# xj361685640/fdtd3d

Hardware: AMD Instinct MI355X
Metric: Mcells/sec (whole node), 3D vacuum 1024^3 grid at 1/2/4/8 MI355X (higher is better)
Workload: dtype fp32; 1 GPU; model=fdtd3d 3D Yee leapfrog, vacuum, point dipole (BASELINE.json headline), grid=1024x1024x1024, global_batch=1, seq_len=1073741824, parallelism=domain-decomposition 1x1x1 (dp1-equivalent ranks), backend=hip

## Files before the change

### fdtd3d_amd/csrc/capi.h

```cpp
#pragma once

#include <stdint.h>

extern "C" {
int fdtd_abi_version();

int fdtd_update_e3d_f32(float* ex, float* ey, float* ez, const float* hx, const float* hy, const float* hz,
                        const float* cbx, const float* cby, const float* cbz, double cb, int nx, int ny, int nz,
                        const int* boxes, int xchunk, void* stream);
int fdtd_update_h3d_f32(float* hx, float* hy, float* hz, const float* ex, const float* ey, const float* ez,
                        const float* dbx, const float* dby, const float* dbz, double db, int nx, int ny, int nz,
                        const int* boxes, int xchunk, void* stream);
int fdtd_update_e3d_f64(double* ex, double* ey, double* ez, const double* hx, const double* hy, const double* hz,
                        const double* cbx, const double* cby, const double* cbz, double cb, int nx, int ny, int nz,
                        const int* boxes, int xchunk, void* stream);
int fdtd_update_h3d_f64(double* hx, double* hy, double* hz, const double* ex, const double* ey, const double* ez,
                        const double* dbx, const double* dby, const double* dbz, double db, int nx, int ny, int nz,
                        const int* boxes, int xchunk, void* stream);
int fdtd_update_e3d_v4_f32(float* ex, float* ey, float* ez, const float* hx, const float* hy, const float* hz,
                           const float* cbx, const float* cby, const float* cbz, double cb, int nx, int ny, int nz,
                           const int* boxes, int xchunk, void* stream);
int fdtd_update_e3d_cpml_v4_f32(float* ex, float* ey, float* ez, const float* hx, const float* hy, const float* hz,
                                const float* cbx, const float* cby, const float* cbz, double cb, int nx, int ny,
                                int nz, const int* boxes, int xchunk, const void* const* cp, const int* ci,
// ... 21 lines not shown
int fdtd_inc_e_f32(float* einc, const float* hinc, int n, double c, double src, void* stream);
int fdtd_inc_e_f64(double* einc, const double* hinc, int n, double c, double src, void* stream);
int fdtd_inc_h_f32(const float* einc, float* hinc, int n, double c, void* stream);
int fdtd_inc_h_f64(const double* einc, double* hinc, int n, double c, void* stream);
int fdtd_tfsf_apply_f32(float* target, const long long* off, const long long* i0, const float* w0, const float* w1,
                        const float* coef, const int* ijk, int n, const float* inc, const int* box, void* stream);
int fdtd_tfsf_apply_f64(double* target, const long long* off, const long long* i0, const double* w0,
                        const double* w1, const double* coef, const int* ijk, int n, const double* inc,
                        const int* box, void* stream);
int fdtd_update_h3d_v4_f32(float* hx, float* hy, float* hz, const float* ex, const float* ey, const float* ez,
                           const float* dbx, const float* dby, const float* dbz, double db, int nx, int ny, int nz,
                           const int* boxes, int xchunk, void* stream);
int fdtd_fused3d_f32(const float* const* ein, const float* const* hin, float* const* eout, float* const* hout,
                     const float* const* cbs, const float* const* dbs, double cb, double db, int nx, int ny, int nz,
                     const int* boxes, int xchunk, long long src_off, int src_comp, double src_val, void* s);
int fdtd_fused3d_f64(const double* const* ein, const double* const* hin, double* const* eout,
                     double* const* hout, const double* const* cbs, const double* const* dbs, double cb, double db,
                     int nx, int ny, int nz, const int* boxes, int xchunk, long long src_off, int src_comp,
                     double src_val, void* s);
int fdtd_fused3d_v4_f32(const float* const* ein, const float* const* hin, float* const* eout, float* const* hout,
                        const float* const* cbs, const float* const* dbs, double cb, double db, int nx, int ny,
                        int nz, const int* boxes, int xchunk, long long src_off, int src_comp, double src_val,
                        void* s);

struct FdtdTbOpts {
  int vec;
  int rows;
  int xcd;
  int mrows;
  int variant;
  int mr_shape;
  int dr_shape;
  int half64;
};
int fdtd_tb_opts_size();
int fdtd_tb3d_v4_f32(const float* const* ein, const float* const* hin, float* const* eout, float* const* hout,
                     const float* const* cbs, const float* const* dbs, double cb, double db, int nx, int ny, int nz,
                     const int* boxes, const int* obox, int xchunk, int steps, const int* src, const double* src_vals,
                     const FdtdTbOpts* opts, void* stream);
int fdtd_tb_max_steps();
int fdtd_tb3d_ext_f32(const float* const* ein, const float* const* hin, float* const* eout, float* const* hout,
                      const void* ce4, const int* ebox, const void* ch4, const int* hbox, double cb, double db,
                      int nx, int ny, int nz, const int* boxes, const int* obox, int xchunk, int steps,
                      const int* src, const double* src_vals, const void* tf, const float* gtab,
                      const FdtdTbOpts* opts, void* stream);
int fdtd_box_pack_f32(float* const* fields, float* buf, int ncomp, int ny, int nz, const int* box, void* s);
int fdtd_box_pack_f64(double* const* fields, double* buf, int ncomp, int ny, int nz, const int* box, void* s);
int fdtd_box_unpack_f32(float* const* fields, const float* buf, int ncomp, int ny, int nz, const int* box, void* s);
int fdtd_box_unpack_f64(double* const* fields, const double* buf, int ncomp, int ny, int nz, const int* box, void* s);
int fdtd_box_xfer_f32(float* const* src, float* const* dst, int ncomp, int ny, int nz, const int* box, void* s);
int fdtd_box_xfer_f64(double* const* src, double* const* dst, int ncomp, int ny, int nz, const int* box, void* s);
int fdtd_tb3d_amp_f32(const float* const* ein, const float* const* hin, float* const* eout, float* const* hout,
                      double cb, double db, int nx, int ny, int nz, const int* boxes, const int* obox, int xchunk,
                      int steps, const int* src, const double* src_vals, float* const* amp, const int* aboxes,
                      double accuracy, unsigned* counts, const FdtdTbOpts* opts, void* stream);
int fdtd_tb3d_drude_f32(const float* const* ein, const float* const* hin, float* const* eout, float* const* hout,
                        double cb, double db, int nx, int ny, int nz, const int* boxes, const int* obox, int xchunk,
                        int steps, const int* src, const double* src_vals, const int* bbox, void* const* sin,
                        void* const* sout, const void* lut, int nid, double cbd, const FdtdTbOpts* opts, void* stream);
int fdtd_tfdev_size();
int fdtd_tfsf_pass_f32(float* einc, float* hinc, int n, double ce, double ch, const double* src_vals, int steps,
                       int reach, int nE, int nH, const int* I0, const float* W0, const float* W1, const float* C,
                       float* gtab, void* stream);
int fdtd_tfsf_table_f32(const float* esrc, const float* hsrc, float* einc, float* hinc, int n, double ce, double ch,
                        const double* src_vals, int steps, int reach, int nE, int nH, const int* I0, const float* W0,
                        const float* W1, const float* C, float* gtab, void* stream);
// ... 108 lines not shown
```

### fdtd3d_amd/csrc/host_native.cpp

```cpp
#include "host_native.h"

#include <algorithm>
#include <cmath>
#include <cstdio>
#include <cstring>
#include <fstream>
#include <limits>
#include <tuple>

namespace fdtd {

double halo_cost(const Int3& size, const Int3& topo) {
  double chunk[3];
  for (int a = 0; a < 3; ++a) chunk[a] = (double)size[a] / topo[a];
  double cost = 0;
  for (int a = 0; a < 3; ++a) {
    if (topo[a] <= 1) continue;
    double other = 1;
    for (int b = 0; b < 3; ++b)
      if (b != a) other *= chunk[b];
    cost += (topo[a] > 2 ? 2 : 1) * other;
  }
  return cost;
}

Int3 optimal_topology(const Int3& size, int p, const std::vector<int>& axes) {
  auto allowed = [&](int a) { return std::find(axes.begin(), axes.end(), a) != axes.end(); };
  Int3 best = {p, 1, 1};
  bool have = false;
  std::tuple<double, int, int, int, int> bestkey;
  for (int pass = 0; pass < 2 && !have; ++pass)
  for (int px = 1; px <= p; ++px) {
    if (p % px) continue;
// ... 234 lines not shown
                                                                         const int* act, int T, int* out, int cap) {
  fdtd::Box6 a, k, dm;
  for (int q = 0; q < 6; ++q) {
    a[q] = alloc[q];
    k[q] = K[q];
    dm[q] = Dm[q];
  }
  const bool ac[3] = {act[0] != 0, act[1] != 0, act[2] != 0};
  std::vector<std::vector<fdtd::Box6>> shells;
  std::vector<fdtd::Box6> copy;
  if (T < 1 || !fdtd::hybrid_windows(a, k, dm, T, ac, {size[0], size[1], size[2]}, shells, copy)) return -1;
  int n = 0;
  auto put = [&](const std::vector<fdtd::Box6>& v) {
    if (n + 1 + 6 * (int)v.size() > cap) return false;
    out[n++] = (int)v.size();
    for (const auto& b : v)
      for (int q = 0; q < 6; ++q) out[n++] = b[q];
    return true;
  };
  for (const auto& v : shells)
    if (!put(v)) return -2;
  if (!put(copy)) return -2;
  return n;
}

extern "C" __attribute__((visibility("default"))) void fdtd_optimal_topology(const int* size, int nprocs,
                                                                                const int* axes, int naxes,
                                                                                int* out) {
  fdtd::Int3 s = {size[0], size[1], size[2]};
  std::vector<int> ax(axes, axes + naxes);
  fdtd::Int3 t = fdtd::optimal_topology(s, nprocs, ax);
  for (int a = 0; a < 3; ++a) out[a] = t[a];
}
```

### fdtd3d_amd/csrc/tb3d_mr.h

```cpp
#pragma once

#include <cstdio>
#include <cstdlib>
#include <type_traits>

#include "capi.h"
#include "common.h"
#include "tfsf_dev.h"

namespace tb3d {

constexpr int TBW = 16;

template <int V>
struct VT;
template <>
struct VT<1> {
  typedef float f __attribute__((ext_vector_type(1)));
  typedef unsigned u __attribute__((ext_vector_type(1)));
};
template <>
struct VT<2> {
  typedef float f __attribute__((ext_vector_type(2)));
  typedef unsigned u __attribute__((ext_vector_type(2)));
};
template <>
struct VT<4> {
  typedef float f __attribute__((ext_vector_type(4)));
  typedef unsigned u __attribute__((ext_vector_type(4)));
};

__device__ __forceinline__ float lane_up(float v) {
  return __builtin_bit_cast(float, __builtin_amdgcn_update_dpp(0, __builtin_bit_cast(int, v), 0x138, 0xf, 0xf, false));
}
__device__ __forceinline__ float lane_dn(float v) {
  return __builtin_bit_cast(float, __builtin_amdgcn_update_dpp(0, __builtin_bit_cast(int, v), 0x130, 0xf, 0xf, false));
}

struct TbSrc {
  float v[8];
// ... 83 lines not shown
}

template <int V>
__device__ __forceinline__ typename VT<V>::f zm1(const typename VT<V>::f& v, float s) {
  typename VT<V>::f r;
  r[0] = s;
#pragma unroll
  for (int q = 1; q < V; ++q) r[q] = v[q - 1];
  return r;
}
template <int V>
__device__ __forceinline__ typename VT<V>::f zp1(const typename VT<V>::f& v, float s) {
  typename VT<V>::f r;
#pragma unroll
  for (int q = 0; q < V - 1; ++q) r[q] = v[q + 1];
  r[V - 1] = s;
  return r;
}

template <int V>
struct F3 {
  typename VT<V>::f x, y, z;
};

template <int T, int V, int R, int FX, int PFD, bool DEFER, int NW>
__global__ __launch_bounds__(64 * NW) void k_tb3d_mr(
    const float* __restrict__ exi, const float* __restrict__ eyi, const float* __restrict__ ezi,
    const float* __restrict__ hxi, const float* __restrict__ hyi, const float* __restrict__ hzi,
    float* __restrict__ exo, float* __restrict__ eyo, float* __restrict__ ezo,
    float* __restrict__ hxo, float* __restrict__ hyo, float* __restrict__ hzo,
    const float4* __restrict__ ce4, const float4* __restrict__ ch4, Box3 BE, Box3 BH, float cb,
    float db, int nx, int ny, int nz, Box3 bex, Box3 bey, Box3 bez, Box3 bhx, Box3 bhy, Box3 bhz, Box3 O,
    int xchunk, int src_i, int src_j, int src_k, int src_comp, TbSrc sv, int xcd_swz,
    const TfDev* __restrict__ tf, const float* __restrict__ gtab, AmpDev amp, DrDev dr) {
  constexpr int PC = FX & 3;
  constexpr bool TFS = FX & 4;
  constexpr bool AMP = FX & 8;
  constexpr bool DRU = FX & 16;
  static_assert(!AMP || (FX == 8 && V == 1 && T <= 3), "amplitude mode: scalar lanes, alone, T <= 3");
  static_assert(!DRU || FX == 16, "Drude box: alone");
  static_assert(V == 1 || !FX, "sparse coefficients / TF/SF: scalar lanes");
  constexpr bool PCE = PC & 1, PCH = PC & 2;
  static_assert(R * V <= 4, "mask bit field holds 7 boxes x R rows x V cells");
  typedef typename VT<V>::f vec;
  constexpr int HL = (T + V - 1) / V;
  constexpr int TBZ = (64 - 2 * HL) * V;
  constexpr int ROWS = NW * R;
  constexpr unsigned VM = (1u << V) - 1u;
  __shared__ vec sX[2][4][NW][64];
  const int lane = threadIdx.x;
  const int w = __builtin_amdgcn_readfirstlane(threadIdx.y);
  typedef const __attribute__((address_space(4))) TfDev* TfPtr;
  const TfPtr TFc = (TfPtr)tf;

  int tz = blockIdx.x, ty = blockIdx.y, tx = blockIdx.z;
  if (xcd_swz & 1) {
    const int gx = gridDim.x, gy = gridDim.y;
    const int n = gx * gy * (int)gridDim.z;
    const int p = blockIdx.x + gx * (blockIdx.y + gy * blockIdx.z);
    const int n8 = n & ~7;
    const int q = p < n8 ? (p & 7) * (n8 >> 3) + (p >> 3) : p;
    const int pz = (xcd_swz >> 8) & 0xff, py = (xcd_swz >> 16) & 0xff;
    if (pz > 0 && py > 0) {
      tx = q / (gx * gy);
      const int r = q - tx * gx * gy;
      const int band = r / (py * gx);
      const int h = min(py, gy - band * py);
      const int rb = r - band * py * gx;
      const int col = rb / (pz * h);
      const int wdt = min(pz, gx - col * pz);
      const int e = rb - col * pz * h;
      tz = col * pz + e % wdt;
      ty = band * py + e / wdt;
    } else {
      tz = q % gx;
      ty = (q / gx) % gy;
      tx = q / (gx * gy);
    }
  }
  const int kb = (O.lo[2] & ~(V - 1)) - HL * V + TBZ * tz + V * lane;
  const int jw = O.lo[1] - T + (ROWS - 2 * T) * ty + R * w;
  const int i0 = O.lo[0] + tx * xchunk;
  const int i1 = min(i0 + xchunk, O.hi[0]);
  const bool kin = kb >= 0 && kb < nz;
  const bool lane_own = lane >= HL && lane < 64 - HL;
  const size_t plane = (size_t)ny * nz;
  unsigned roff[R];
  unsigned mbits = 0;
  const Box3* bx[7] = {&bex, &bey, &bez, &bhx, &bhy, &bhz, &O};
#pragma unroll
  for (int r = 0; r < R; ++r) {
    const int j = jw + r;
    const int t = R * w + r;
    const bool ld_ok = kin && j >= 0 && j < ny;
    roff[r] = ld_ok ? (unsigned)(j * nz + kb) * 4u : 0xF0000000u;
    const bool own = ld_ok && lane_own && t >= T && t < ROWS - T;
#pragma unroll
    for (int n = 0; n < 7; ++n) {
      const bool ok = n < 6 ? ld_ok : own;
      mbits |= (ok ? kmaskv<V>(*bx[n], j, kb) : 0u) << ((r * 7 + n) * V);
    }
  }
  const int rdn = w > 0 ? w - 1 : 0;
  const int rup = w < NW - 1 ? w + 1 : NW - 1;
  const vec zero = (vec)(0.f);
  const vec cbv = (vec)(cb), dbv = (vec)(db);
  unsigned upd_bits = 0;
#pragma unroll
  for (int r = 0; r < R; ++r) upd_bits |= ((1u << (6 * V)) - 1u) << (r * 7 * V);
  const bool tile_all = __all((mbits & upd_bits) == upd_bits);

  unsigned eoff[R], hoff[R];
  unsigned inb = 0;
  const int bez_n = BE.hi[2] - BE.lo[2], bhz_n = BH.hi[2] - BH.lo[2];
  const size_t eplane = (size_t)(BE.hi[1] - BE.lo[1]) * bez_n * 16u;
  const size_t hplane = (size_t)(BH.hi[1] - BH.lo[1]) * bhz_n * 16u;
// ... 551 lines not shown
      for (int r = 0; r < R; ++r) Hs[r] = Hc[r];
    } else {
      if constexpr (TFS)
        store_plane(X, Ep[T - 1], Hc);
      else
        store_plane(X, En, Hc);
    }
  }
  if (DEFER) {
    F3<V> Es[R];
#pragma unroll
    for (int r = 0; r < R; ++r) Es[r] = Ep[T - 1][r];
    store_plane(i1 + T - 1, Es, Hs);
  }
  };
  if (tile_all && !(xcd_swz & 2))
    run(std::true_type{});
  else
    run(std::false_type{});
  if constexpr (AMP) {
#pragma unroll
    for (int l = 0; l < T; ++l) {
      unsigned v = acnt[l];
#pragma unroll
      for (int d = 32; d > 0; d >>= 1) v += __shfl_xor(v, d, 64);
      if (lane == 0 && v) atomicAdd(amp.counts + l, v);
    }
  }
}


inline FdtdTbOpts tb_opts(const FdtdTbOpts* p) {
  FdtdTbOpts o = { 0,  0,  0,  0,  4,  0,  0,
                   1};
  if (!p) return o;
  o.vec = (p->vec == 2 || p->vec == 4) ? p->vec : 0;
  o.rows = (p->rows == 1 || p->rows == 2) ? p->rows : 0;
  o.xcd = p->xcd ? 1 : 0;
  o.mrows = (p->mrows == 1 || p->mrows == 2) ? p->mrows : 0;
  o.variant = p->variant & 15;
  o.mr_shape = (p->mr_shape == 1 || p->mr_shape == 2) ? p->mr_shape : 0;
  o.dr_shape = p->dr_shape == 1 ? 1 : 0;
  o.half64 = p->half64 ? 1 : 0;
  return o;
}

inline int tb_patch_bits() {
  static const int bits = [] {
    const char* e = getenv("FDTD3D_TB_PATCH");
    int pz = 0, py = 0;
    if (e && sscanf(e, "%dx%d", &pz, &py) == 2 && pz > 0 && py > 0 && pz < 256 && py < 256)
      return (pz << 8) | (py << 16);
    return 0;
  }();
  return bits;
}

template <int T, int V, int R, int FX, int NW = TBW>
int launch_tb_mr(const FdtdTbOpts& o, const float* const* ein, const float* const* hin, float* const* eout,
                 float* const* hout, const float4* ce4, const float4* ch4, const Box3& BE, const Box3& BH, float cb,
                 float db, int nx, int ny, int nz, const Box3* b, const Box3& O, int xchunk, const int* src,
                 const TbSrc& sv, const TfDev* tf, const float* gtab, const AmpDev& amp, hipStream_t s,
                 const DrDev& dr = DrDev{}) {
  constexpr int HL = (T + V - 1) / V;
  constexpr int TBZ = (64 - 2 * HL) * V;
  dim3 grid(cdiv(O.hi[2] - (O.lo[2] & ~(V - 1)), TBZ), cdiv(O.hi[1] - O.lo[1], NW * R - 2 * T),
            cdiv(O.hi[0] - O.lo[0], xchunk));
  const int noallin = (o.variant >> 3) & 1;
  const int swz = (o.variant & 4) ? (1 | (noallin << 1) | tb_patch_bits()) : (noallin << 1);
#define MR_LAUNCH(PFD, DEFER)                                                                                 \
  k_tb3d_mr<T, V, R, FX, PFD, DEFER, NW><<<grid, dim3(64, NW), 0, s>>>(                                     \
      ein[0], ein[1], ein[2], hin[0], hin[1], hin[2], eout[0], eout[1], eout[2], hout[0], hout[1], hout[2], \
      ce4, ch4, BE, BH, cb, db, nx, ny, nz, b[0], b[1], b[2], b[3], b[4], b[5],                             \
      O, xchunk, src[0], src[1], src[2], src[3], sv, swz, tf, gtab, amp, dr)
  if constexpr (FX != 0) {
    MR_LAUNCH(1, false);
  } else {
    switch (o.variant & 3) {
      case 0: MR_LAUNCH(1, false); break;
      case 1: MR_LAUNCH(1, true); break;
      case 2: MR_LAUNCH(2, false); break;
      default: MR_LAUNCH(2, true); break;
    }
  }
#undef MR_LAUNCH
  FDTD_RETURN_LAUNCH_STATUS();
}

}
```

### fdtd3d_amd/csrc/yee3d_tb.hip

```cpp

#include <cstdio>
#include <cstdlib>
#include <type_traits>

#include "common.h"

#include "tb3d_mr.h"

namespace {

using namespace tb3d;

template <int T, int V, int R, bool PERCELL>
__global__ __launch_bounds__(64 * TBW) void k_tb3d(
    const float* __restrict__ exi, const float* __restrict__ eyi, const float* __restrict__ ezi,
    const float* __restrict__ hxi, const float* __restrict__ hyi, const float* __restrict__ hzi,
    float* __restrict__ exo, float* __restrict__ eyo, float* __restrict__ ezo,
    float* __restrict__ hxo, float* __restrict__ hyo, float* __restrict__ hzo,
    const float* __restrict__ cbx, const float* __restrict__ cby, const float* __restrict__ cbz,
    const float* __restrict__ dbx, const float* __restrict__ dby, const float* __restrict__ dbz, float cb,
    float db, int nx, int ny, int nz, Box3 bex, Box3 bey, Box3 bez, Box3 bhx, Box3 bhy, Box3 bhz, Box3 O,
    int xchunk, int src_i, int src_j, int src_k, int src_comp, TbSrc sv, int xcd_swz) {
  typedef typename VT<V>::f vec;
  constexpr bool PF = V == 2;
// ... 103 lines not shown
      }
      const int ph = pe - 1;
      const float ey_k3 = lane_dn(Ep[l].y[0]);
      const float ex_k3 = lane_dn(Ep[l].x[0]);
      F3<V> Hn;
      const vec chx = coef(dbx, bhx, ph, mhx, mchx, dbv);
      Hn.x = Hp[l].x + chx * ((zp1<V>(Ep[l].y, ey_k3) - Ep[l].y) - (ez_jn - Ep[l].z));
      const vec chy = coef(dby, bhy, ph, mhy, mchy, dbv);
      Hn.y = Hp[l].y + chy * ((En.z - Ep[l].z) - (zp1<V>(Ep[l].x, ex_k3) - Ep[l].x));
      const vec chz = coef(dbz, bhz, ph, mhz, mchz, dbv);
      Hn.z = Hp[l].z + chz * ((ex_jn - Ep[l].x) - (En.y - Ep[l].y));
      Ec = Ep[l];
      Ep[l] = En;
      Hp[l] = Hc;
      Hc = Hn;
    }
    if (mo) {
      const int pe = X - T + 1;
      if (pe >= i0 && pe < i1) {
        bst<V>(plane_rsrc(exo, pe, nx, plane), row, En.x, mo);
        bst<V>(plane_rsrc(eyo, pe, nx, plane), row, En.y, mo);
        bst<V>(plane_rsrc(ezo, pe, nx, plane), row, En.z, mo);
      }
      const int ph = X - T;
      if (ph >= i0 && ph < i1) {
        bst<V>(plane_rsrc(hxo, ph, nx, plane), row, Hc.x, mo);
        bst<V>(plane_rsrc(hyo, ph, nx, plane), row, Hc.y, mo);
        bst<V>(plane_rsrc(hzo, ph, nx, plane), row, Hc.z, mo);
      }
    }
  }
}

int g_num_cus = 0;
int pick_xchunk(long long tiles_yz, int nxo, int T, int wg_per_cu = 1) {
  if (g_num_cus <= 0) {
    int dev = 0, n = 0;
    if (hipGetDevice(&dev) == hipSuccess &&
        hipDeviceGetAttribute(&n, hipDeviceAttributeMultiprocessorCount, dev) == hipSuccess && n > 0)
      g_num_cus = n;
    else
      g_num_cus = 256;
  }
  if (nxo <= 0) return 1;
  const long long slots = (long long)g_num_cus * wg_per_cu;
  auto search = [&](int cap, long long* rounds_out) {
    long long best_cost = -1, best_rounds = 1;
    int best = nxo;
    for (int k = 1; k <= 256; ++k) {
      const int xc = (nxo + k - 1) / k;
      if (xc > cap) continue;
      const long long chunks = (nxo + xc - 1) / xc;
      const long long rounds = (tiles_yz * chunks + slots - 1) / slots;
      const long long cost = rounds * (xc + 2LL * T);
      if (best_cost < 0 || cost < best_cost) {
        best_cost = cost;
        best = xc;
        best_rounds = rounds;
      }
      if (xc == 1) break;
    }
    *rounds_out = best_rounds;
    return best;
  };
  long long rounds = 1;
  const int best = search(nxo, &rounds);
  static int cap = -1;
  if (cap < 0) {
    const char* e = getenv("FDTD3D_TB_XCAP");
    cap = (e && atoi(e) > 0) ? atoi(e) : 192;
  }
  if (rounds >= 2 && best > cap) return search(cap, &rounds);
  return best;
}

template <int T, int V, int R, bool PERCELL>
int launch_tb(const float* const* ein, const float* const* hin, float* const* eout, float* const* hout,
              const float* const* cbs, const float* const* dbs, float cb, float db, int nx, int ny, int nz,
              const Box3* b, const Box3& O, int xchunk, const int* src, const TbSrc& sv, hipStream_t s, int xcd) {
  constexpr int HL = (T + V - 1) / V;
  constexpr int TBZ = (64 / R - 2 * HL) * V;
  dim3 grid(cdiv(O.hi[2] - (O.lo[2] & ~(V - 1)), TBZ), cdiv(O.hi[1] - O.lo[1], TBW * R - 2 * T),
            cdiv(O.hi[0] - O.lo[0], xchunk));
  k_tb3d<T, V, R, PERCELL><<<grid, dim3(64, TBW), 0, s>>>(
      ein[0], ein[1], ein[2], hin[0], hin[1], hin[2], eout[0], eout[1], eout[2], hout[0], hout[1], hout[2],
      cbs[0], cbs[1], cbs[2], dbs[0], dbs[1], dbs[2], cb, db, nx, ny, nz, b[0], b[1], b[2], b[3], b[4], b[5], O,
      xchunk, src[0], src[1], src[2], src[3], sv, xcd);
  FDTD_RETURN_LAUNCH_STATUS();
}

template <int T, int V, int R>
int launch_tb_pc(bool pc, const float* const* ein, const float* const* hin, float* const* eout,
                 float* const* hout, const float* const* cbs, const float* const* dbs, float cb, float db, int nx,
                 int ny, int nz, const Box3* b, const Box3& O, int xchunk, const int* src, const TbSrc& sv,
                 hipStream_t s, int xcd) {
  return pc ? launch_tb<T, V, R, true>(ein, hin, eout, hout, cbs, dbs, cb, db, nx, ny, nz, b, O, xchunk, src, sv, s,
                                       xcd)
            : launch_tb<T, V, R, false>(ein, hin, eout, hout, cbs, dbs, cb, db, nx, ny, nz, b, O, xchunk, src, sv,
                                        s, xcd);
}

constexpr int MR_AUTO_ROWS = 2;

const int kNoBox[6] = {0, 0, 0, 0, 0, 0};
static int tb_amp_shape() {
  static const int v = [] {
// ... 16 lines not shown
      if (o.dr_shape == 1) return launch_tb_mr<T, 1, 1, 16, 16>(MR_ARGS);
      return launch_tb_mr<T, 1, 2, 16, 8>(MR_ARGS);
    }
    return (int)hipErrorInvalidValue;
  }
  if (fx == 8) {
    if constexpr (T <= 3) {
      if (o.mr_shape == 1) return launch_tb_mr<T, 1, 4, 8, 8>(MR_ARGS);
      if (tb_amp_shape() == 2) return launch_tb_mr<T, 1, 2, 8, 8>(MR_ARGS);
      return launch_tb_mr<T, 1, 2, 8>(MR_ARGS);
    }
    return (int)hipErrorInvalidValue;
  }
  if constexpr (T <= 5) {
    switch (fx) {
      case 1: return launch_tb_mr<T, 1, 2, 1>(MR_ARGS);
      case 2: return launch_tb_mr<T, 1, 2, 2>(MR_ARGS);
      case 3: return launch_tb_mr<T, 1, 2, 3>(MR_ARGS);
      case 4: return launch_tb_mr<T, 1, 2, 4>(MR_ARGS);
      case 5: return launch_tb_mr<T, 1, 2, 5>(MR_ARGS);
      case 6: return launch_tb_mr<T, 1, 2, 6>(MR_ARGS);
      case 7: return launch_tb_mr<T, 1, 2, 7>(MR_ARGS);
    }
  } else {
    if (fx) return (int)hipErrorInvalidValue;
  }
  if (o.mr_shape == 1) return launch_tb_mr<T, 1, 4, 0, 8>(MR_ARGS);
  if constexpr (T <= 5)
    if (o.mr_shape == 2) return launch_tb_mr<T, 1, 2, 0, 8>(MR_ARGS);
  return launch_tb_mr<T, 1, 2, 0>(MR_ARGS);
#undef MR_ARGS
}

int tb_mr_xchunk(int fx, const FdtdTbOpts& o, const Box3& O, int steps) {
  const long long gz = cdiv(O.hi[2] - O.lo[2], 64 - 2 * steps);
  const bool amp16 = fx == 8 && o.mr_shape != 1 && tb_amp_shape() == 2;
  const bool rows16 = fx == 16 || amp16 || (fx == 0 && o.mr_shape == 2 && steps <= 5);
  const long long gy = cdiv(O.hi[1] - O.lo[1], (rows16 ? 16 : TBW * 2) - 2 * steps);
  return pick_xchunk(gz * gy, O.hi[0] - O.lo[0], steps, ((fx == 0 && o.mr_shape >= 1) || amp16) ? 2 : 1);
}

int tb_mr_dispatch(int fx, const FdtdTbOpts& o, const float* const* ein, const float* const* hin,
                   float* const* eout, float* const* hout, const float4* ce4, const float4* ch4, const Box3& BE,
                   const Box3& BH, float cb, float db, int nx, int ny, int nz, const Box3* b, const Box3& O,
                   int xchunk, int steps, const int* src, const TbSrc& sv, const TfDev* tf, const float* gtab,
                   const AmpDev& amp, hipStream_t s, const DrDev& dr = DrDev{}) {
  if (xchunk <= 0 && (fx & 4)) {
    static const int tfx = [] {
      const char* e = getenv("FDTD3D_TF_XCHUNK");
      return e ? atoi(e) : 0;
    }();
    if (tfx > 0) xchunk = tfx;
  }
  if (xchunk <= 0) xchunk = tb_mr_xchunk(fx, o, O, steps);
#define MR_ARGS \
  fx, o, ein, hin, eout, hout, ce4, ch4, BE, BH, cb, db, nx, ny, nz, b, O, xchunk, src, sv, tf, gtab, amp, s, dr
  switch (steps) {
    case 1: return launch_tb_mr_sel<1>(MR_ARGS);
    case 2: return launch_tb_mr_sel<2>(MR_ARGS);
    case 3: return launch_tb_mr_sel<3>(MR_ARGS);
    case 4: return launch_tb_mr_sel<4>(MR_ARGS);
    case 5: return launch_tb_mr_sel<5>(MR_ARGS);
    case 6: return launch_tb_mr_sel<6>(MR_ARGS);
  }
#undef MR_ARGS
  return (int)hipErrorInvalidValue;
}

template <typename R>
struct LineSrc {
  R v[8];
};
template <typename R>
__global__ __launch_bounds__(1024) void k_tfsf_pass(R* __restrict__ einc, R* __restrict__ hinc, int n, R ce, R ch,
                                                    LineSrc<R> sv, int T, int reach, int nE, int nH,
                                                    const int* __restrict__ I0, const R* __restrict__ W0,
                                                    const R* __restrict__ W1, const R* __restrict__ C,
                                                    R* __restrict__ gtab, const R* __restrict__ esrc,
                                                    const R* __restrict__ hsrc) {
  const int tid = threadIdx.x;
  const int ld = nE + nH;
  const int m = min(n, reach);
  if (esrc) {
    for (int i = tid; i < min(n, reach + 1); i += blockDim.x) {
      einc[i] = esrc[i];
      hinc[i] = hsrc[i];
    }
// ... 215 lines not shown
```

### fdtd3d_amd/ops/hip_ops.py

```python

from __future__ import annotations

import ctypes
import os
import threading
from typing import Dict, List, Optional, Sequence, Tuple

import torch

from ..layout.yee import YeeLayout
from ..models.regions import RegionLevel
from .coef import Coef
from .hip_lib import HipError, _check, _ptr, _stream, c_double, c_int, c_ll, c_vp
from .hip_monitors import HipMonitorOps

Box = Tuple[Tuple[int, int, int], Tuple[int, int, int]]

_LIB = None
TB_MAX_STEPS = 6
TB_MAX_STEPS_F64 = 5
TB2D_MAX_STEPS = 8
TB2D_MAX_STEPS_F64 = 8
TB2D_MODES = {("Ez",): (0, ("Ez",), ("Hx", "Hy")), ("Ex", "Ey"): (1, ("Ex", "Ey"), ("Hz",))}
_LIB_PATH = os.environ.get("FDTD3D_HIP_LIB") or os.path.join(os.path.dirname(os.path.dirname(os.path.abspath(__file__))),
# ... 17 lines not shown
    global _LIB
    if _LIB is not None:
        return _LIB
    if not os.path.exists(_LIB_PATH) and build_if_missing:
        from .build import build
        build(exe=False)
    if not os.path.exists(_LIB_PATH):
        raise HipError("libfdtd3d_hip.so not found at %s: run `python -m fdtd3d_amd.ops.build`" % _LIB_PATH)
    _LIB = ctypes.CDLL(_LIB_PATH)
    _LIB.fdtd_abi_version.restype = c_int
    return _LIB


def available() -> bool:
    try:
        load_library(build_if_missing=False)
    except (HipError, OSError):
        return False
    return torch.cuda.is_available()


def _box_arr(boxes: Sequence[Box]):
    vals = []
    for b in boxes:
        vals += list(b[0]) + list(b[1])
    return (c_int * len(vals))(*vals)


def _empty(b: Box) -> bool:
    return any(b[1][d] <= b[0][d] for d in range(3))


class TbOpts(ctypes.Structure):
    _fields_ = [(n, c_int) for n in ("vec", "rows", "xcd", "mrows", "variant", "mr_shape", "dr_shape", "half64")]


class _RecFn:
    __slots__ = ("f", "ops")

    def __init__(self, f, ops):
        self.f, self.ops = f, ops

    def __call__(self, *args):
        rec = self.ops._rec
        if rec is not None:
            rec.append((self.f, args))
        return self.f(*args)


_SETTERS = ("fdtd_set_chain_v4", "fdtd_set_chain_split", "fdtd_set_fused_rows", "fdtd_set_lowdim_wgs")


class _LibProxy:

    def __init__(self, lib, ops):
        self.raw, self._ops, self._w = lib, ops, {}

    def __getattr__(self, name):
        w = self._w.get(name)
        if w is None:
            f = getattr(self.raw, name)
            w = self._w[name] = f if name in _SETTERS else _RecFn(f, self._ops)
        return w


_EMPTY_CPML = ((c_vp * 45)(), (c_int * 36)())

# ... 683 lines not shown
        if einc.numel() != hinc.numel():
            raise HipError("tfsf_pass: E / H lines of different length")
        vals8 = (c_double * 8)(*(list(src_vals) + [0.0] * (8 - T)))
        tail = (c_int(T), c_int(min(einc.numel(), reach)), c_int(sets.n_e), c_int(sets.n_h), _ptr(sets.i0),
                _ptr(sets.w0), _ptr(sets.w1), _ptr(sets.c), _ptr(g), _stream())
        if dry:
            scr = sets.__dict__.setdefault("scratch_lines", {})
            sl = scr.get(slot)
            if sl is None or sl[0].numel() != einc.numel():
                sl = scr[slot] = (torch.zeros_like(einc), torch.zeros_like(hinc))
            rc = getattr(self.lib, "fdtd_tfsf_table_" + sfx)(_ptr(einc), _ptr(hinc), _ptr(sl[0]), _ptr(sl[1]),
                                                             c_int(einc.numel()), c_double(ce), c_double(ch), vals8,
                                                             *tail)
        else:
            rc = getattr(self.lib, "fdtd_tfsf_pass_" + sfx)(_ptr(einc), _ptr(hinc), c_int(einc.numel()), c_double(ce),
                                                            c_double(ch), vals8, *tail)
        _check(rc, "tfsf_pass")
        self.launches += 1
        return g

    def _check_tfdev(self, sets) -> None:
        if self._tfdev_size != 4 * sets.dev.numel():
            raise HipError("TfDev layout mismatch (%d vs %d bytes)" % (self._tfdev_size, 4 * sets.dev.numel()))

    def _tb_opts(self, steps: int = 0, thin_obox: Optional[Box] = None):
        mr, mr_shape = self.tb_mrows, self.tb_mr_shape
        if (thin_obox is not None and mr == 0 and self.tb_thin_single_row and steps <= 4
                and thin_obox[1][1] - thin_obox[0][1] <= 8):
            if self.tb_thin_mr16:
                mr_shape = 2
            else:
                mr = 1
        return ctypes.byref(TbOpts(self.tb_vec, self.tb_rows, self.tb_xcd, mr, self.tb_variant, mr_shape,
                                   self.tb_dr_shape, self.tb64_half))

    @staticmethod
    def _check_inside(op: str, boxes: Sequence[Box], shape, nd: int = 3, empty_too: bool = False) -> None:
        for b in boxes:
            if (empty_too or not _empty(b)) and any(b[0][d] < 0 or b[1][d] > shape[d] for d in range(nd)):
                raise HipError("%s: box %s outside array %s" % (op, b, shape))

    @staticmethod
    def _tb_source(op: str, sources, comps, shape, nd: int = 3):
        src, vals = [-1] * (nd + 1), [0.0] * 8
        if sources is not None and any(s is not None for s in sources):
            first = next(s for s in sources if s is not None)
            comp, idx = first[0], tuple(first[1])
            if comp not in comps:
                raise HipError("%s: point source on %s only, got %s" % (op, "/".join(comps), comp))
            if not all(0 <= idx[d] < shape[d] for d in range(nd)):
                raise HipError("%s: source index %s outside array %s" % (op, idx, shape))
            for l, s in enumerate(sources):
                if s is None or s[0] != comp or tuple(s[1]) != idx:
                    raise HipError("%s: the source must be the same point at every step" % op)
                vals[l] = float(s[2])
            src = list(idx[:nd]) + [comps.index(comp)]
        return (c_int * len(src))(*src), (c_double * 8)(*vals)

    def _tb3d_pass(self, op: str, fin, fout, boxes: Dict[str, Box], obox: Box, cb: Dict[str, Coef],
                   more_boxes: Sequence[Box] = (), uniform: str = ""):
        E, H = ("Ex", "Ey", "Ez"), ("Hx", "Hy", "Hz")
        shape = tuple(fin["Ex"].shape)
        if self.dtype == torch.float32 and shape[2] % 4 != 0:
            raise HipError("fp32 %s needs nz %% 4 == 0, got %s" % (op, shape))
        for c in E + H:
            self._check_tensor(fin[c], shape)
            self._check_tensor(fout[c], shape)
# ... 151 lines not shown
                ptrs += [None] * len(names)
                sv[kind] = cb[names[0]].scalar
                if any(cb[c].scalar != sv[kind] for c in names):
                    raise HipError("tb_step: scalar coefficients must agree per kind")
        cs = (c_vp * 3)(*ptrs)
        cbv, dbv = sv["E"], sv["H"]
        src, vals = self._tb_source("2D tb_step", sources, comps, shape, nd=2)
        two = lambda names, f: (c_vp * 2)(*([f[c].data_ptr() for c in names] + [None] * (2 - len(names))))
        rc = self.fn("tb2d")(c_int(mode), two(E, fin), two(H, fin), two(E, fout), two(H, fout), cs,
                                    c_double(cbv), c_double(dbv), c_int(shape[0]), c_int(shape[1]),
                                    _box_arr([boxes[c] for c in comps]), _box_arr([obox]), c_int(self.tb_xchunk),
                                    c_int(steps), src, vals, _stream())
        _check(rc, "tb2d")
        self.launches += 1

    @property
    def tb2d_max_steps(self) -> int:
        return TB2D_MAX_STEPS if self.dtype == torch.float32 else TB2D_MAX_STEPS_F64

    @property
    def tb_max_steps(self) -> int:
        return TB_MAX_STEPS if self.dtype == torch.float32 else TB_MAX_STEPS_F64

    tb_xchunk = int(os.environ.get("FDTD3D_TB_XCHUNK", "0"))
    tb_vec = 0
    tb_rows = 0
    tb_xcd = 0
    tb_variant = 4
    tb_mrows = 0
    tb_thin_single_row = True
    tb_thin_mr16 = os.environ.get("FDTD3D_TB_THIN_MR16", "0") == "1"
    tb_sparse = True
    tb_mr_shape = int(os.environ.get("FDTD3D_TB_MR_SHAPE", "0"))
    tb64_half = int(os.environ.get("FDTD3D_TB64_HALF", "1"))

    def chain_update(self, kind: str, boxes: Dict[str, Box], F: Dict[str, torch.Tensor], upml: Dict[str, dict],
                     p: int, drude: bool, plain_form: bool = False, plain: Optional[Dict[str, Box]] = None,
                     cb: Optional[Dict[str, Coef]] = None, rows=None) -> None:
        if rows is not None and (not drude or cb is None):
            raise HipError("chain_update rows: dispersive launches with the plain coefficients only")
        comps = list(boxes.keys())
        if len(comps) != 3:
            raise HipError("chain_update launches the three components of a kind together")
        shape = tuple(F[comps[0]].shape)
        P, S, I = [], [], []
        any_box = False
        for c in comps:
            st = upml[c]
            pr = st["plain"]["prof"] if plain_form else st["prof"]
            b = boxes[c]
            terms = self.layout.curl_terms(c)
            if len(terms) != 2:
                raise HipError("chain_update is the 3D chain (2 curl terms per component)")
            if not _empty(b):
                any_box = True
                self._check_stencil_box(kind, c, b, shape)
            D = st["D"][p]
            aux = [D[-1], D[0], D[1] if drude else None]
            if drude:
                D1 = st["D1"][p]
                aux += [D1[2], D1[0], D1[1]]
            else:
                aux += [None, None, None]
            dbox = ((0, 0, 0), (0, 0, 0))
            if isinstance(D[0], RegionLevel):
                parts = [None if t is None else t.part(b) for t in aux]
# ... 187 lines not shown
```

Measured before the change: 296,800 Mcells/s.

## Add mixed full-column/x-chunked workgroup schedule for temporal-blocking kernel

Flattens the temporal-blocking launch grid to 1D and adds a scheduler that can give most yz tiles a full x column while splitting only the leftover tiles into x chunks to fill the last wave. This targets tail-wave imbalance and the 2T halo recompute that uniform x-chunking adds. The default mode (1) keeps uniform chunking, though slot counting now assumes two workgroups per CU for some FX=0, NW=8 shapes where it previously depended on mr_shape. Tile indexing moves to division and modulo in the kernel.

```diff
diff --git a/fdtd3d_amd/csrc/capi.h b/fdtd3d_amd/csrc/capi.h
--- a/fdtd3d_amd/csrc/capi.h
+++ b/fdtd3d_amd/csrc/capi.h
@@ -77,6 +77,10 @@
   int mr_shape;
   int dr_shape;
   int half64;
+  int slots;
+  int xsched;
+  int xs_cap;
+  int xs_rounds;
 };
 int fdtd_tb_opts_size();
 int fdtd_tb3d_v4_f32(const float* const* ein, const float* const* hin, float* const* eout, float* const* hout,
diff --git a/fdtd3d_amd/csrc/host_native.cpp b/fdtd3d_amd/csrc/host_native.cpp
--- a/fdtd3d_amd/csrc/host_native.cpp
+++ b/fdtd3d_amd/csrc/host_native.cpp
@@ -1,4 +1,6 @@
 #include "host_native.h"
+
+#include "tb_xsched.h"
 
 #include <algorithm>
 #include <cmath>
@@ -299,3 +301,14 @@
   fdtd::Int3 t = fdtd::optimal_topology(s, nprocs, ax);
   for (int a = 0; a < 3; ++a) out[a] = t[a];
 }
+
+extern "C" __attribute__((visibility("default"))) int fdtd_tb_xsched(long long tiles_yz, int nxo, int T,
+                                                                    long long slots, int cap, int mode,
+                                                                    int last_cap, int last_rounds, int* out) {
+  const tb3d::XSched s = tb3d::xsched_pick(tiles_yz, nxo, T, slots, cap, mode, last_cap, last_rounds);
+  out[0] = s.full;
+  out[1] = s.rest;
+  out[2] = s.chunks;
+  out[3] = s.xc;
+  return tb3d::xchunk_uniform(tiles_yz, nxo, T, slots, cap, nullptr);
+}
diff --git a/fdtd3d_amd/csrc/tb3d_mr.h b/fdtd3d_amd/csrc/tb3d_mr.h
--- a/fdtd3d_amd/csrc/tb3d_mr.h
+++ b/fdtd3d_amd/csrc/tb3d_mr.h
@@ -6,6 +6,7 @@
 
 #include "capi.h"
 #include "common.h"
+#include "tb_xsched.h"
 #include "tfsf_dev.h"
 
 namespace tb3d {
@@ -155,7 +156,8 @@
     const float4* __restrict__ ce4, const float4* __restrict__ ch4, Box3 BE, Box3 BH, float cb,
     float db, int nx, int ny, int nz, Box3 bex, Box3 bey, Box3 bez, Box3 bhx, Box3 bhy, Box3 bhz, Box3 O,
     int xchunk, int src_i, int src_j, int src_k, int src_comp, TbSrc sv, int xcd_swz,
-    const TfDev* __restrict__ tf, const float* __restrict__ gtab, AmpDev amp, DrDev dr) {
+    const TfDev* __restrict__ tf, const float* __restrict__ gtab, AmpDev amp, DrDev dr, int xs_full, int xs_rest,
+    int gtz, int gty) {
   constexpr int PC = FX & 3;
   constexpr bool TFS = FX & 4;
   constexpr bool AMP = FX & 8;
@@ -176,17 +178,22 @@
   typedef const __attribute__((address_space(4))) TfDev* TfPtr;
   const TfPtr TFc = (TfPtr)tf;
 
-  int tz = blockIdx.x, ty = blockIdx.y, tx = blockIdx.z;
+  const int gx = gtz, gy = gty;
+  const bool cut = (int)blockIdx.x >= xs_full;
+  const int p = (int)blockIdx.x - (cut ? xs_full : 0);
+  int q = p;
   if (xcd_swz & 1) {
-    const int gx = gridDim.x, gy = gridDim.y;
-    const int n = gx * gy * (int)gridDim.z;
-    const int p = blockIdx.x + gx * (blockIdx.y + gy * blockIdx.z);
+    const int n = cut ? (int)gridDim.x - xs_full : xs_full;
     const int n8 = n & ~7;
-    const int q = p < n8 ? (p & 7) * (n8 >> 3) + (p >> 3) : p;
+    q = p < n8 ? (p & 7) * (n8 >> 3) + (p >> 3) : p;
+  }
+  const int tx = __builtin_amdgcn_readfirstlane(cut ? q / xs_rest : 0);
+  const int tile = cut ? xs_full + q - tx * xs_rest : q;
+  int tz = tile % gx, ty = tile / gx;
+  if (xcd_swz & 1) {
     const int pz = (xcd_swz >> 8) & 0xff, py = (xcd_swz >> 16) & 0xff;
     if (pz > 0 && py > 0) {
-      tx = q / (gx * gy);
-      const int r = q - tx * gx * gy;
+      const int r = tile;
       const int band = r / (py * gx);
       const int h = min(py, gy - band * py);
       const int rb = r - band * py * gx;
@@ -195,16 +202,12 @@
       const int e = rb - col * pz * h;
       tz = col * pz + e % wdt;
       ty = band * py + e / wdt;
-    } else {
-      tz = q % gx;
-      ty = (q / gx) % gy;
-      tx = q / (gx * gy);
     }
   }
   const int kb = (O.lo[2] & ~(V - 1)) - HL * V + TBZ * tz + V * lane;
   const int jw = O.lo[1] - T + (ROWS - 2 * T) * ty + R * w;
   const int i0 = O.lo[0] + tx * xchunk;
-  const int i1 = min(i0 + xchunk, O.hi[0]);
+  const int i1 = cut ? min(i0 + xchunk, O.hi[0]) : O.hi[0];
   const bool kin = kb >= 0 && kb < nz;
   const bool lane_own = lane >= HL && lane < 64 - HL;
   const size_t plane = (size_t)ny * nz;
@@ -822,7 +825,7 @@
 
 inline FdtdTbOpts tb_opts(const FdtdTbOpts* p) {
   FdtdTbOpts o = { 0,  0,  0,  0,  4,  0,  0,
-                   1};
+                   1,  0,  XSCHED_DEFAULT,  0,  1};
   if (!p) return o;
   o.vec = (p->vec == 2 || p->vec == 4) ? p->vec : 0;
   o.rows = (p->rows == 1 || p->rows == 2) ? p->rows : 0;
@@ -832,7 +835,30 @@
   o.mr_shape = (p->mr_shape == 1 || p->mr_shape == 2) ? p->mr_shape : 0;
   o.dr_shape = p->dr_shape == 1 ? 1 : 0;
   o.half64 = p->half64 ? 1 : 0;
+  o.slots = (p->slots > 0 && p->slots <= (1 << 20)) ? p->slots : 0;
+  o.xsched = (p->xsched >= 1 && p->xsched <= 3) ? p->xsched : XSCHED_DEFAULT;
+  o.xs_cap = p->xs_cap > 0 ? p->xs_cap : 0;
+  o.xs_rounds = p->xs_rounds == 2 ? 2 : 1;
   return o;
+}
+
+inline int tb_num_cus() {
+  static const int cus = [] {
+    int dev = 0, n = 0;
+    if (hipGetDevice(&dev) == hipSuccess &&
+        hipDeviceGetAttribute(&n, hipDeviceAttributeMultiprocessorCount, dev) == hipSuccess && n > 0)
+      return n;
+    return 256;
+  }();
+  return cus;
+}
+
+inline int tb_xcap() {
+  static const int cap = [] {
+    const char* e = getenv("FDTD3D_TB_XCAP");
+    return (e && atoi(e) > 0) ? atoi(e) : 192;
+  }();
+  return cap;
 }
 
 inline int tb_patch_bits() {
@@ -854,15 +880,26 @@
                  const DrDev& dr = DrDev{}) {
   constexpr int HL = (T + V - 1) / V;
   constexpr int TBZ = (64 - 2 * HL) * V;
-  dim3 grid(cdiv(O.hi[2] - (O.lo[2] & ~(V - 1)), TBZ), cdiv(O.hi[1] - O.lo[1], NW * R - 2 * T),
-            cdiv(O.hi[0] - O.lo[0], xchunk));
+  const int gtz = cdiv(O.hi[2] - (O.lo[2] & ~(V - 1)), TBZ), gty = cdiv(O.hi[1] - O.lo[1], NW * R - 2 * T);
+  const long long tiles = (long long)gtz * gty;
+  const int nxo = O.hi[0] - O.lo[0];
+  constexpr int WPC = ((FX == 0 || (FX == 8 && R == 2)) && NW == 8) ? 2 : 1;
+  const long long slots = o.slots > 0 ? o.slots : (long long)tb_num_cus() * WPC;
+  const XSched xs = xchunk > 0 ? xsched_uniform(tiles, nxo, xchunk)
+                               : xsched_pick(tiles, nxo, T, slots, tb_xcap(), FX == 0 ? o.xsched : 1, o.xs_cap,
+                                             o.xs_rounds);
+  const long long nwg = xs.full + (long long)xs.rest * xs.chunks;
+  if (tiles <= 0 || nxo <= 0) return 0;
+  if (nwg > 0x7fffffffLL) return (int)hipErrorInvalidValue;
+  dim3 grid((unsigned)nwg);
+  const int xs_rest = xs.rest > 0 ? xs.rest : 1;
   const int noallin = (o.variant >> 3) & 1;
   const int swz = (o.variant & 4) ? (1 | (noallin << 1) | tb_patch_bits()) : (noallin << 1);
 #define MR_LAUNCH(PFD, DEFER)                                                                                 \
   k_tb3d_mr<T, V, R, FX, PFD, DEFER, NW><<<grid, dim3(64, NW), 0, s>>>(                                     \
       ein[0], ein[1], ein[2], hin[0], hin[1], hin[2], eout[0], eout[1], eout[2], hout[0], hout[1], hout[2], \
       ce4, ch4, BE, BH, cb, db, nx, ny, nz, b[0], b[1], b[2], b[3], b[4], b[5],                             \
-      O, xchunk, src[0], src[1], src[2], src[3], sv, swz, tf, gtab, amp, dr)
+      O, xs.xc, src[0], src[1], src[2], src[3], sv, swz, tf, gtab, amp, dr, xs.full, xs_rest, gtz, gty)
   if constexpr (FX != 0) {
     MR_LAUNCH(1, false);
   } else {
diff --git a/fdtd3d_amd/csrc/tb_xsched.h b/fdtd3d_amd/csrc/tb_xsched.h
--- /dev/null
+++ b/fdtd3d_amd/csrc/tb_xsched.h
@@ -0,0 +1,78 @@
+#pragma once
+
+namespace tb3d {
+
+inline int xchunk_uniform(long long tiles_yz, int nxo, int T, long long slots, int cap, long long* rounds_out) {
+  if (rounds_out) *rounds_out = 1;
+  if (nxo <= 0) return 1;
+  if (slots < 1) slots = 1;
+  auto search = [&](int lim, long long* rounds) {
+    long long best_cost = -1, best_rounds = 1;
+    int best = nxo;
+    for (int k = 1; k <= 256; ++k) {
+      const int xc = (nxo + k - 1) / k;
+      if (xc > lim) continue;
+      const long long chunks = (nxo + xc - 1) / xc;
+      const long long r = (tiles_yz * chunks + slots - 1) / slots;
+      const long long cost = r * (xc + 2LL * T);
+      if (best_cost < 0 || cost < best_cost) {
+        best_cost = cost;
+        best = xc;
+        best_rounds = r;
+      }
+      if (xc == 1) break;
+    }
+    *rounds = best_rounds;
+    return best;
+  };
+  long long rounds = 1, capped = 1;
+  const int best = search(nxo, &rounds);
+  if (rounds_out) *rounds_out = rounds;
+  if (rounds >= 2 && best > cap) return search(cap, &capped);
+  return best;
+}
+
+struct XSched {
+  int full;
+  int rest;
+  int chunks;
+  int xc;
+};
+
+inline XSched xsched_uniform(long long tiles_yz, int nxo, int xc) {
+  if (xc < 1) xc = 1;
+  return XSched{0, (int)tiles_yz, nxo > 0 ? (nxo + xc - 1) / xc : 1, xc};
+}
+
+constexpr int XSCHED_DEFAULT = 1;
+
+inline XSched xsched_pick(long long tiles_yz, int nxo, int T, long long slots, int cap, int mode, int last_cap,
+                          int last_rounds) {
+  if (slots < 1) slots = 1;
+  long long rounds = 1;
+  const int uxc = xchunk_uniform(tiles_yz, nxo, T, slots, cap, &rounds);
+  const XSched u = xsched_uniform(tiles_yz, nxo, uxc);
+  if (mode != 2 && mode != 3) return u;
+  if (nxo <= 0 || tiles_yz <= 0) return u;
+  if (mode == 2 && (rounds < 2 || tiles_yz < slots)) return u;
+  long long whole = tiles_yz / slots;
+  const long long cut_rounds = (last_rounds == 2 && whole >= 2) ? 2 : 1;
+  whole -= whole > 0 ? cut_rounds - 1 : 0;
+  XSched m;
+  m.full = (int)(whole * slots);
+  m.rest = (int)(tiles_yz - m.full);
+  long long k = m.rest > 0 ? (cut_rounds * slots) / m.rest : 1;
+  if (last_cap > 0 && (nxo + last_cap - 1) / last_cap > k) k = (nxo + last_cap - 1) / last_cap;
+  if (k < 1) k = 1;
+  if (k > nxo) k = nxo;
+  m.xc = (int)((nxo + k - 1) / k);
+  m.chunks = (nxo + m.xc - 1) / m.xc;
+  if (mode == 2) {
+    const long long cost_m = whole * (nxo + 2LL * T) + (((long long)m.rest * m.chunks + slots - 1) / slots) * (m.xc + 2LL * T);
+    const long long cost_u = ((tiles_yz * u.chunks + slots - 1) / slots) * (u.xc + 2LL * T);
+    if (cost_m > cost_u) return u;
+  }
+  return m;
+}
+
+}
diff --git a/fdtd3d_amd/csrc/yee3d_tb.hip b/fdtd3d_amd/csrc/yee3d_tb.hip
--- a/fdtd3d_amd/csrc/yee3d_tb.hip
+++ b/fdtd3d_amd/csrc/yee3d_tb.hip
@@ -159,46 +159,8 @@
   }
 }
 
-int g_num_cus = 0;
 int pick_xchunk(long long tiles_yz, int nxo, int T, int wg_per_cu = 1) {
-  if (g_num_cus <= 0) {
-    int dev = 0, n = 0;
-    if (hipGetDevice(&dev) == hipSuccess &&
-        hipDeviceGetAttribute(&n, hipDeviceAttributeMultiprocessorCount, dev) == hipSuccess && n > 0)
-      g_num_cus = n;
-    else
-      g_num_cus = 256;
-  }
-  if (nxo <= 0) return 1;
-  const long long slots = (long long)g_num_cus * wg_per_cu;
-  auto search = [&](int cap, long long* rounds_out) {
-    long long best_cost = -1, best_rounds = 1;
-    int best = nxo;
-    for (int k = 1; k <= 256; ++k) {
-      const int xc = (nxo + k - 1) / k;
-      if (xc > cap) continue;
-      const long long chunks = (nxo + xc - 1) / xc;
-      const long long rounds = (tiles_yz * chunks + slots - 1) / slots;
-      const long long cost = rounds * (xc + 2LL * T);
-      if (best_cost < 0 || cost < best_cost) {
-        best_cost = cost;
-        best = xc;
-        best_rounds = rounds;
-      }
-      if (xc == 1) break;
-    }
-    *rounds_out = best_rounds;
-    return best;
-  };
-  long long rounds = 1;
-  const int best = search(nxo, &rounds);
-  static int cap = -1;
-  if (cap < 0) {
-    const char* e = getenv("FDTD3D_TB_XCAP");
-    cap = (e && atoi(e) > 0) ? atoi(e) : 192;
-  }
-  if (rounds >= 2 && best > cap) return search(cap, &rounds);
-  return best;
+  return xchunk_uniform(tiles_yz, nxo, T, (long long)tb_num_cus() * wg_per_cu, tb_xcap(), nullptr);
 }
 
 template <int T, int V, int R, bool PERCELL>
@@ -281,14 +243,6 @@
 #undef MR_ARGS
 }
 
-int tb_mr_xchunk(int fx, const FdtdTbOpts& o, const Box3& O, int steps) {
-  const long long gz = cdiv(O.hi[2] - O.lo[2], 64 - 2 * steps);
-  const bool amp16 = fx == 8 && o.mr_shape != 1 && tb_amp_shape() == 2;
-  const bool rows16 = fx == 16 || amp16 || (fx == 0 && o.mr_shape == 2 && steps <= 5);
-  const long long gy = cdiv(O.hi[1] - O.lo[1], (rows16 ? 16 : TBW * 2) - 2 * steps);
-  return pick_xchunk(gz * gy, O.hi[0] - O.lo[0], steps, ((fx == 0 && o.mr_shape >= 1) || amp16) ? 2 : 1);
-}
-
 int tb_mr_dispatch(int fx, const FdtdTbOpts& o, const float* const* ein, const float* const* hin,
                    float* const* eout, float* const* hout, const float4* ce4, const float4* ch4, const Box3& BE,
                    const Box3& BH, float cb, float db, int nx, int ny, int nz, const Box3* b, const Box3& O,
@@ -301,7 +255,7 @@
     }();
     if (tfx > 0) xchunk = tfx;
   }
-  if (xchunk <= 0) xchunk = tb_mr_xchunk(fx, o, O, steps);
+  if (xchunk <= 0) xchunk = 0;
 #define MR_ARGS \
   fx, o, ein, hin, eout, hout, ce4, ch4, BE, BH, cb, db, nx, ny, nz, b, O, xchunk, src, sv, tf, gtab, amp, s, dr
   switch (steps) {
diff --git a/fdtd3d_amd/ops/hip_ops.py b/fdtd3d_amd/ops/hip_ops.py
--- a/fdtd3d_amd/ops/hip_ops.py
+++ b/fdtd3d_amd/ops/hip_ops.py
@@ -73,7 +73,8 @@
 
 
 class TbOpts(ctypes.Structure):
-    _fields_ = [(n, c_int) for n in ("vec", "rows", "xcd", "mrows", "variant", "mr_shape", "dr_shape", "half64")]
+    _fields_ = [(n, c_int) for n in ("vec", "rows", "xcd", "mrows", "variant", "mr_shape", "dr_shape", "half64",
+                                     "slots", "xsched", "xs_cap", "xs_rounds")]
 
 
 class _RecFn:
@@ -823,7 +824,8 @@
             else:
                 mr = 1
         return ctypes.byref(TbOpts(self.tb_vec, self.tb_rows, self.tb_xcd, mr, self.tb_variant, mr_shape,
-                                   self.tb_dr_shape, self.tb64_half))
+                                   self.tb_dr_shape, self.tb64_half, self.tb_slots, self.tb_xsched, self.tb_xs_cap,
+                                   self.tb_xs_rounds))
 
     @staticmethod
     def _check_inside(op: str, boxes: Sequence[Box], shape, nd: int = 3, empty_too: bool = False) -> None:
@@ -1041,6 +1043,10 @@
     tb_thin_mr16 = os.environ.get("FDTD3D_TB_THIN_MR16", "0") == "1"
     tb_sparse = True
     tb_mr_shape = int(os.environ.get("FDTD3D_TB_MR_SHAPE", "0"))
+    tb_xsched = int(os.environ.get("FDTD3D_TB_XSCHED", "0"))
+    tb_slots = 0
+    tb_xs_cap = int(os.environ.get("FDTD3D_TB_XS_CAP", "0"))
+    tb_xs_rounds = int(os.environ.get("FDTD3D_TB_XS_ROUNDS", "1"))
     tb64_half = int(os.environ.get("FDTD3D_TB64_HALF", "1"))
 
     def chain_update(self, kind: str, boxes: Dict[str, Box], F: Dict[str, torch.Tensor], upml: Dict[str, dict],
```

Result: no change. 299,400 Mcells/s, median of 6 (+0.9%).
